# PeterFWS/Structure-PLP-SLAM

Measured on AMD Instinct MI355X. Metric: frames/sec ORB+LSD extract+match, 640x480 TUM-RGBD, 1/2/4/8 GPU, higher is better.
Workload: dtype u8

## Files before the change

### structure-plp-slam_amd/csrc/orb_context.hip

```cpp
#include <hip/hip_runtime.h>

#include <algorithm>
#include <cstdio>
#include <cstring>
#include <mutex>
#include <string>
#include <vector>

#include "blur_tile.hpp"
#include "orb_device.hpp"
#include "xcd_map.hpp"
#include "plp_common.hpp"
#include "quadtree_model.hpp"

namespace plp {
void launch_quadtree(hipStream_t st, const LevelDev* d_lv, int n_levels, int n_cells_total, const uint32_t* cell_cand,
                     const int32_t* cell_count, int32_t* sel, int32_t* sel_count, int total_sel_cap, uint32_t* qt_scratch,
                     size_t qt_scratch_frame_stride, int32_t* status, int B, int max_quota);
size_t quadtree_scratch_bytes_per_frame(const LevelDev* h_lv, int n_levels);
}

using namespace plp;

struct plp_orb {
    HostPinned pin;
    plp_orb_params p{};
    std::vector<float> rects;
    int device = 0;
    hipStream_t stream = nullptr;
    OrbScaleTables st;
    OrbGeometry geo;
    std::vector<LevelDev> h_lv;
    int total_blur_tiles = 0;
    DevBuf d_lv, d_cells, d_rs;
    ResizeDev rs{};
    int capB = 0;
    DevBuf pyr, blur, l0copy, cell_cand, cell_count, sel, sel_count, status, qt_scratch, d_mask;
    size_t l0copy_frame_stride = 0, qt_frame_stride = 0;
    int max_quota = 0;
    DevBuf s_kps, s_desc, s_counts;
    DevBuf stereo_corr, stereo_stage;
    int s_cap = 0;
    bool mask_is_initialized = false;
    std::vector<uint8_t> rect_mask;
    int rect_mask_rows = 0, rect_mask_cols = 0;
    bool rect_mask_uploaded = false;
    DevBuf d_rect_mask;
    int last_B = 0;
    OrbPlanes last_planes{};
    hipStream_t last_stream = nullptr;
    bool profiling = false;
    hipEvent_t ev[8] = {};
    double stage_ms[7] = {0, 0, 0, 0, 0, 0, 0};
    long stage_batches = 0;
    std::mutex mu;
};

namespace {

plp_status validate(const plp_orb_params* p) {
    if (!p) return set_error(PLP_ERR_INVALID_ARG, "params is NULL");
    if (p->num_levels == 0 || p->num_levels > (uint32_t)kMaxLevels) return set_error(PLP_ERR_INVALID_ARG, "num_levels must be in [1,16]");
    if (!(p->scale_factor > 1.0f)) return set_error(PLP_ERR_INVALID_ARG, "scale_factor must be > 1");
    if (p->n_mask_rects < 0 || (p->n_mask_rects > 0 && !p->mask_rects)) return set_error(PLP_ERR_INVALID_ARG, "mask_rects");
    for (int i = 0; i < p->n_mask_rects; ++i) {
        const float* v = p->mask_rects + 4 * i;
        if (v[0] >= v[1]) return set_error(PLP_ERR_INVALID_ARG, "x_max must be greater than x_min");
        if (v[2] >= v[3]) return set_error(PLP_ERR_INVALID_ARG, "y_max must be greater than x_min");
    }
    return PLP_OK;
}

void reinitialize(plp_orb* c) {
    c->st = make_scale_tables(c->p.max_num_keypts, c->p.scale_factor, c->p.num_levels);
    c->geo = OrbGeometry{};
}

plp_status build_geometry_impl(plp_orb* c, int rows, int cols);

plp_status build_geometry(plp_orb* c, int rows, int cols) {
    if (c->geo.rows == rows && c->geo.cols == cols && c->geo.n_levels == (int)c->p.num_levels) return PLP_OK;
    const plp_status s = build_geometry_impl(c, rows, cols);
    if (s != PLP_OK) { c->geo = OrbGeometry{}; c->h_lv.clear(); c->capB = 0; }
    return s;
}

plp_status build_geometry_impl(plp_orb* c, int rows, int cols) {
    const int nl = (int)c->p.num_levels;
    {
        OrbGeometry g = make_geometry(rows, cols, c->st, nl);
        for (int l = 0; l < nl; ++l)
            if (g.lv[l].w <= 2 * kOrbBorder + 6 || g.lv[l].h <= 2 * kOrbBorder + 6)
                return set_error(PLP_ERR_INVALID_ARG, "image too small for the requested pyramid (level narrower than 45 px)");
        if (cols - 2 * kOrbBorder > 4095 || rows - 2 * kOrbBorder > 4095)
            return set_error(PLP_ERR_UNSUPPORTED, "images larger than 4133 px are not supported (12-bit candidate packing)");
        c->geo = std::move(g);
    }
    c->h_lv.assign(nl, LevelDev{});
    c->total_blur_tiles = 0;
    size_t qt_off = 0;
    int max_cells = 0;
    for (int l = 0; l < nl; ++l) {
        const LevelGeom& G = c->geo.lv[l];
        LevelDev& L = c->h_lv[l];
        L.w = G.w; L.h = G.h; L.pitch = G.pitch; L.off = G.off;
        L.blur_tiles = ((G.w + 127) / 128) * ((G.h + plp::kBlurTH - 1) / plp::kBlurTH);
        L.blur_tiles_x_magic = plp::plp_div_magic((uint32_t)((G.w + 127) / 128), (uint64_t)L.blur_tiles);
        c->total_blur_tiles += L.blur_tiles;
        L.scale = c->st.sf[l];
        L.sel_base = G.sel_base; L.sel_cap = G.sel_cap;
        L.cell_base = G.cell_base; L.n_cells = G.n_cell_rows * G.n_cell_cols;
        L.quota = (int)c->st.quota[l];
        c->max_quota = l == 0 ? L.quota : std::max(c->max_quota, L.quota);
        L.n_init_x = G.n_init_x; L.delta_x = G.delta_x; L.delta_y = G.delta_y;
        L.qt_cap = std::min(std::max(L.n_cells, 1) * kCellCap, 65535);
        L.qt_off = qt_off;
        qt_off += (size_t)L.qt_cap * 20;
        const int extent = (int)std::ceil(std::max(G.delta_x, G.delta_y)) + 1;
        int t1 = 0;
        while ((1 << t1) < extent) ++t1;
        const int d_eff = std::min(t1 + 2, kQtDepth);
        const int n_init = G.n_init_x * G.n_init_y;
        int nb = 0;
        while ((1 << nb) < n_init) ++nb;
        L.sort_lo = 2 * (kQtDepth - d_eff);
        L.sort_hi = 2 * kQtDepth + nb;
        if (L.n_cells > 2048 || 3 * L.quota + 8 > kQtMaxNodesLdsSmallBlock || n_init > 32)
            return set_error(PLP_ERR_UNSUPPORTED, "frame/keypoint budget exceeds the quadtree kernel limits (quota per level <= 2010, 2048 cells per level, 32 initial nodes)");
        max_cells = std::max(max_cells, L.n_cells);
    }
    if (3 * c->max_quota + 8 > kQtMaxNodesLds && max_cells > 1024)
        return set_error(PLP_ERR_UNSUPPORTED, "frame/keypoint budget exceeds the quadtree kernel limits (a quota above 1960 per level needs levels of at most 1024 cells)");
    PLP_HIP(c->d_lv.upload(c->h_lv.data(), sizeof(LevelDev) * nl, c->stream));
    PLP_HIP(c->d_cells.upload(c->geo.cells.data(), sizeof(CellDesc) * c->geo.cells.size(), c->stream));
    const ResizeTables& R = c->geo.rs;
    const size_t nc = R.xofs0.size(), nr = R.yofs0.size();
    std::vector<int16_t> blob;
    blob.reserve(4 * nc + 4 * nr + 8);
    auto push = [&](const std::vector<int16_t>& v) { size_t o = blob.size(); blob.insert(blob.end(), v.begin(), v.end()); return o; };
    const size_t o0 = push(R.xofs0), o1 = push(R.xofs1), o2 = push(R.a0), o3 = push(R.a1);
    const size_t o4 = push(R.yofs0), o5 = push(R.yofs1), o6 = push(R.b0), o7 = push(R.b1);
    if (blob.empty()) blob.push_back(0);
    PLP_HIP(c->d_rs.upload(blob.data(), blob.size() * 2, c->stream));
    const int16_t* base = (const int16_t*)c->d_rs.p;
    c->rs.xofs0 = base + o0; c->rs.xofs1 = base + o1; c->rs.a0 = base + o2; c->rs.a1 = base + o3;
    c->rs.yofs0 = base + o4; c->rs.yofs1 = base + o5; c->rs.b0 = base + o6; c->rs.b1 = base + o7;
    for (int l = 0; l < nl; ++l) { c->rs.col_base[l] = R.col_base[l]; c->rs.row_base[l] = R.row_base[l]; }
    c->capB = 0;
    PLP_HIP(hipStreamSynchronize(c->stream));
    return PLP_OK;
}

plp_status ensure_capacity(plp_orb* c, int B) {
    if (B <= c->capB) return PLP_OK;
    const OrbGeometry& g = c->geo;
    const size_t n_cells = g.cells.size();
    c->l0copy_frame_stride = ((size_t)g.lv[0].pitch * g.rows + 255) / 256 * 256;
    c->qt_frame_stride = quadtree_scratch_bytes_per_frame(c->h_lv.data(), g.n_levels);
    PLP_HIP(c->pyr.reserve(g.frame_plane_bytes * B));
    PLP_HIP(c->blur.reserve(g.frame_plane_bytes * B));
    PLP_HIP(c->l0copy.reserve(c->l0copy_frame_stride * B));
    PLP_HIP(c->cell_cand.reserve(sizeof(uint32_t) * kCellCap * n_cells * B));
    PLP_HIP(c->cell_count.reserve(sizeof(int32_t) * n_cells * B));
    PLP_HIP(c->sel.reserve(sizeof(int32_t) * g.total_sel_cap * B));
    PLP_HIP(c->sel_count.reserve(sizeof(int32_t) * kMaxLevels * B));
    PLP_HIP(c->status.reserve(sizeof(int32_t) * 4));
    PLP_HIP(c->qt_scratch.reserve(c->qt_frame_stride * B));
    c->capB = B;
    return PLP_OK;
}

void build_rect_mask(plp_orb* c, int rows, int cols) {
    if (c->mask_is_initialized || c->rects.empty()) return;
    if (c->rect_mask.empty()) { c->rect_mask.assign((size_t)rows * cols, 255); c->rect_mask_rows = rows; c->rect_mask_cols = cols; }
    for (size_t i = 0; i + 3 < c->rects.size(); i += 4) {
        const unsigned x0 = (unsigned)std::round((float)cols * c->rects[i]), x1 = (unsigned)std::round((float)cols * c->rects[i + 1]);
        const unsigned y0 = (unsigned)std::round((float)rows * c->rects[i + 2]), y1 = (unsigned)std::round((float)rows * c->rects[i + 3]);
        for (unsigned y = y0; y <= y1 && y < (unsigned)c->rect_mask_rows; ++y)
            for (unsigned x = x0; x <= x1 && x < (unsigned)c->rect_mask_cols; ++x) c->rect_mask[(size_t)y * c->rect_mask_cols + x] = 0;
    }
    c->mask_is_initialized = true;
    c->rect_mask_uploaded = false;
}

plp_status run_batch(plp_orb* c, const uint8_t* d_imgs, int B, int rows, int cols, size_t step, size_t frame_stride,
                     const uint8_t* d_mask, size_t mask_step, size_t mask_frame_stride, plp_keypoint* d_kps, uint8_t* d_desc,
                     int cap, int32_t* d_counts, hipStream_t st) {
    PLP_HIP(hipSetDevice(c->device));
    PLP_TRY(build_geometry(c, rows, cols));
    PLP_TRY(ensure_capacity(c, B));
    const OrbGeometry& g = c->geo;
    const int nl = g.n_levels;

    const bool prof = c->profiling;
    auto mark = [&](int i) { if (prof) (void)hipEventRecord(c->ev[i], st); };
    mark(0);
    OrbPlanes pl{};
    pl.pyr = (uint8_t*)c->pyr.p; pl.pyr_frame_stride = g.frame_plane_bytes;
    const bool aligned = ((uintptr_t)d_imgs % 4 == 0) && (step % 4 == 0) && (frame_stride % 4 == 0);
    if (aligned) { pl.l0 = d_imgs; pl.l0_frame_stride = frame_stride; pl.l0_pitch = (int)step; }
    else {
        for (int f = 0; f < B; ++f)
            PLP_HIP(hipMemcpy2DAsync((uint8_t*)c->l0copy.p + f * c->l0copy_frame_stride, g.lv[0].pitch, d_imgs + f * frame_stride, step,
                                     cols, rows, hipMemcpyDeviceToDevice, st));
        pl.l0 = (const uint8_t*)c->l0copy.p; pl.l0_frame_stride = c->l0copy_frame_stride; pl.l0_pitch = g.lv[0].pitch;
    }
    build_rect_mask(c, rows, cols);
    if (!d_mask && !c->rect_mask.empty()) {
        if (c->rect_mask_rows != rows || c->rect_mask_cols != cols)
            return set_error(PLP_ERR_INVALID_ARG, "rectangle mask was built for a different frame size");
        if (!c->rect_mask_uploaded) {
            PLP_HIP(c->d_rect_mask.upload(c->rect_mask.data(), c->rect_mask.size(), st));
            c->rect_mask_uploaded = true;
        }
        d_mask = (const uint8_t*)c->d_rect_mask.p; mask_step = cols; mask_frame_stride = 0;
    }

    PLP_HIP(hipMemsetAsync(c->status.p, 0, 16, st));
    mark(1);
    for (int l = 1; l < nl; ++l) launch_resize(st, pl, c->h_lv.data(), l, B, c->rs);
    mark(2);
    launch_fast(st, pl, (const CellDesc*)c->d_cells.p, (int)g.cells.size(), (const LevelDev*)c->d_lv.p, B, (int)c->p.ini_fast_thr,
                (int)c->p.min_fast_thr, d_mask, mask_step, mask_frame_stride, (uint32_t*)c->cell_cand.p, (int32_t*)c->cell_count.p);
    mark(3);
    BlurTaps taps{{18, 34, 48, 56, 48, 34, 18}};
    launch_blur(st, pl, (uint8_t*)c->blur.p, g.frame_plane_bytes, (const LevelDev*)c->d_lv.p, nl, c->total_blur_tiles, B, taps, c->h_lv.data());
    mark(4);
    launch_quadtree(st, (const LevelDev*)c->d_lv.p, nl, (int)g.cells.size(), (const uint32_t*)c->cell_cand.p,
                    (const int32_t*)c->cell_count.p, (int32_t*)c->sel.p, (int32_t*)c->sel_count.p, g.total_sel_cap,
                    (uint32_t*)c->qt_scratch.p, c->qt_frame_stride, (int32_t*)c->status.p, B, c->max_quota);
    mark(5);
    UMax um;
    for (int v = 0; v <= kHalfPatch; ++v) um.v[v] = c->st.u_max[v];
    launch_orient_rbrief(st, pl, (const uint8_t*)c->blur.p, g.frame_plane_bytes, (const LevelDev*)c->d_lv.p, nl, (const int32_t*)c->sel.p,
                         (const int32_t*)c->sel_count.p, g.total_sel_cap, um, d_kps, d_desc, cap, d_counts, (int32_t*)c->status.p, B);
    PLP_HIP(hipGetLastError());
    if (prof) {
        mark(6);
        PLP_HIP(hipEventSynchronize(c->ev[6]));
        for (int i = 0; i < 6; ++i) { float ms = 0; PLP_HIP(hipEventElapsedTime(&ms, c->ev[i], c->ev[i + 1])); c->stage_ms[i] += ms; }
        float tot = 0; PLP_HIP(hipEventElapsedTime(&tot, c->ev[0], c->ev[6])); c->stage_ms[6] += tot;
        ++c->stage_batches;
    }
    c->last_B = B; c->last_planes = pl; c->last_stream = st;
    return PLP_OK;
}

}

extern "C" {

void plp_orb_default_params(plp_orb_params* p) {
    if (!p) return;
    p->max_num_keypts = 2000; p->scale_factor = 1.2f; p->num_levels = 8; p->ini_fast_thr = 20; p->min_fast_thr = 7;
    p->mask_rects = nullptr; p->n_mask_rects = 0;
}

plp_status plp_orb_create(const plp_orb_params* params, int device, plp_orb** out) {
    if (!out) return set_error(PLP_ERR_INVALID_ARG, "out is NULL");
    *out = nullptr;
// ... 292 lines not shown
```

### structure-plp-slam_amd/csrc/orb_device.hpp

```cpp
#pragma once
#include <hip/hip_runtime.h>
#include <stdint.h>

#include "../../include/plp_front.h"
#include "orb_tables.hpp"

namespace plp {

constexpr int kQtMaxNodesLds = 5888;
constexpr int kQtMaxNodesLdsSmallBlock = 6040;

struct LevelDev {
    int w, h, pitch;
    int blur_tiles;
    uint32_t blur_tiles_x_magic;
    size_t off;
    float scale;
    int sel_base, sel_cap;
    int cell_base, n_cells;
    int quota;
    int n_init_x;
    double delta_x, delta_y;
    size_t qt_off;
    int qt_cap;
    int sort_lo, sort_hi;
};

struct OrbPlanes {
    const uint8_t* l0; size_t l0_frame_stride; int l0_pitch;
    uint8_t* pyr; size_t pyr_frame_stride;
    __host__ __device__ const uint8_t* level_ptr(int frame, int level, const LevelDev& L) const {
        return level == 0 ? l0 + (size_t)frame * l0_frame_stride : pyr + (size_t)frame * pyr_frame_stride + L.off;
    }
    __host__ __device__ int level_pitch(int level, const LevelDev& L) const { return level == 0 ? l0_pitch : L.pitch; }
};

struct BlurTaps { int k[7]; };
struct UMax { int v[kHalfPatch + 1]; };

struct ResizeDev {
    const int16_t *xofs0, *xofs1, *a0, *a1, *yofs0, *yofs1, *b0, *b1;
    int col_base[kMaxLevels], row_base[kMaxLevels];
};

struct StereoArgs {
    const plp_keypoint *kps_l, *kps_r;
    const uint8_t *desc_l, *desc_r;
    const int32_t *cnt_l, *cnt_r;
    int cap;
    float fxb, tb;
    float inv_scale[kMaxLevels];
    float* x_right; float* depth;
    int32_t* corr;
};
void launch_stereo(hipStream_t st, const OrbPlanes& pl_l, const OrbPlanes& pl_r, const LevelDev* d_lv, const StereoArgs& A, int B);

void launch_resize(hipStream_t st, const OrbPlanes& pl, const LevelDev* h_lv, int level, int B, const ResizeDev& rs);
void launch_fast(hipStream_t st, const OrbPlanes& pl, const CellDesc* d_cells, int n_cells, const LevelDev* d_lv, int B,
                 int ini_thr, int min_thr, const uint8_t* d_mask, size_t mask_step, size_t mask_frame_stride,
                 uint32_t* cell_cand, int32_t* cell_count);
void launch_blur(hipStream_t st, const OrbPlanes& pl, uint8_t* blur, size_t blur_frame_stride, const LevelDev* d_lv,
                 int n_levels, int total_tiles, int B, const BlurTaps& taps, const LevelDev* h_lv = nullptr);
void launch_orient_rbrief(hipStream_t st, const OrbPlanes& pl, const uint8_t* blur, size_t blur_frame_stride,
                          const LevelDev* d_lv, int n_levels, const int32_t* sel, const int32_t* sel_count,
                          int total_sel_cap, const UMax& um, plp_keypoint* kps, uint8_t* desc, int cap, int32_t* counts,
                          int32_t* status, int B);

}
```

### structure-plp-slam_amd/csrc/orb_kernels.hip

```cpp
#include <hip/hip_runtime.h>
#include <stdint.h>

#include "blur_tile.hpp"
#include "plp_barrier.hpp"
#include "orb_device.hpp"
#include "plp_common.hpp"
#include "xcd_map.hpp"

namespace plp {

__device__ __forceinline__ int rs_tab(const int16_t* __restrict__ t, int i) { return *reinterpret_cast<const int16_t*>(reinterpret_cast<const char*>(t) + ((uint32_t)i << 1)); }
constexpr int kRsRows = 44, kRsPitch = 96;

__global__ __launch_bounds__(256) __attribute__((amdgpu_waves_per_eu(7, 8))) void k_resize_linear(const uint8_t* __restrict__ src_base, size_t src_frame_stride,
                                                       int src_pitch, int sw, uint8_t* __restrict__ dst_base,
                                                       size_t dst_frame_stride, int dst_pitch, int dw, int dh,
                                                       const int16_t* __restrict__ xofs0, const int16_t* __restrict__ xofs1,
                                                       const int16_t* __restrict__ a0, const int16_t* __restrict__ a1,
                                                       const int16_t* __restrict__ yofs0, const int16_t* __restrict__ yofs1,
                                                       const int16_t* __restrict__ b0, const int16_t* __restrict__ b1) {
    constexpr int ROWS = 8;
    __shared__ __attribute__((aligned(16))) uint8_t tiles[4 * kRsRows * kRsPitch];
    const int lane = threadIdx.x & 63, wv = __builtin_amdgcn_readfirstlane((int)(threadIdx.x >> 6));
    const int strip_x0 = blockIdx.x * 64, strip_y0 = (blockIdx.y * 4 + wv) * 32;
    if (strip_y0 >= dh) return;
    uint8_t* tile = tiles + wv * (kRsRows * kRsPitch);
    const int strip_x1 = min(strip_x0 + 64, dw) - 1, strip_y1 = min(strip_y0 + 32, dh) - 1;
    const uint8_t* src = src_base + (size_t)blockIdx.z * src_frame_stride;
    uint8_t* dst = dst_base + (size_t)blockIdx.z * dst_frame_stride;
    const int xs = (int)xofs0[strip_x0] & ~15, xe = xofs1[strip_x1];
    const int ys = yofs0[strip_y0], ye = yofs1[strip_y1];
    const int nrows = ye - ys + 1, nchunks = (xe - xs) / 16 + 1;
    const bool staged = nrows <= kRsRows && nchunks * 16 <= kRsPitch;
    if (staged) {
        const bool wide = (((uintptr_t)src | (uintptr_t)src_pitch) & 15) == 0;
        const int c = lane & 7, r0 = lane >> 3;
        if (c < nchunks) {
            const int x = xs + 16 * c;
            if (wide && x + 16 <= src_pitch) {
                constexpr int NT = (kRsRows + 7) / 8;
                uint4 v[NT];
#pragma unroll
                for (int q = 0; q < NT; ++q) v[q] = *reinterpret_cast<const uint4*>(src + (uint32_t)(__mul24(ys + min(r0 + 8 * q, nrows - 1), src_pitch) + x));
#pragma unroll
                for (int q = 0; q < NT; ++q) { const int r = r0 + 8 * q; if (r < nrows) *reinterpret_cast<uint4*>(tile + r * kRsPitch + 16 * c) = v[q]; }
            } else
                for (int r = r0; r < nrows; r += 8) {
                    const uint8_t* g = src + (size_t)(ys + r) * src_pitch + x;
                    uint8_t* t = tile + r * kRsPitch + 16 * c;
                    for (int k = 0; k < 16; ++k) t[k] = x + k < sw ? g[k] : (uint8_t)0;
                }
        }
        __builtin_amdgcn_fence(__ATOMIC_ACQ_REL, "workgroup");
        __builtin_amdgcn_wave_barrier();
    }
    const int dy0 = strip_y0 + (lane >> 4) * ROWS;
    const int dx0 = strip_x0 + (lane & 15) * 4;
    if (dy0 >= dh || dx0 >= dw) return;
    int x0[4], x1[4], wa0[4], wa1[4];
#pragma unroll
    for (int i = 0; i < 4; ++i) {
        const int dx = min(dx0 + i, dw - 1);
        x0[i] = rs_tab(xofs0, dx); x1[i] = rs_tab(xofs1, dx); wa0[i] = rs_tab(a0, dx); wa1[i] = rs_tab(a1, dx);
    }
    if (staged) {
#pragma unroll
        for (int i = 0; i < 4; ++i) { x0[i] -= xs; x1[i] -= xs; }
        int cached_row = -1, hc[4] = {0, 0, 0, 0};
        auto hrow = [&](int y, int (&h)[4]) {
            const uint8_t* S = tile + (y - ys) * kRsPitch;
#pragma unroll
            for (int i = 0; i < 4; ++i) h[i] = S[x0[i]] * wa0[i] + S[x1[i]] * wa1[i];
        };
        uint32_t tyy[ROWS], tbb[ROWS];
#pragma unroll
        for (int r = 0; r < ROWS; ++r) {
            const int dy = min(dy0 + r, dh - 1);
            tyy[r] = (uint32_t)(uint16_t)rs_tab(yofs0, dy) | ((uint32_t)(uint16_t)rs_tab(yofs1, dy) << 16);
            tbb[r] = (uint32_t)(uint16_t)rs_tab(b0, dy) | ((uint32_t)(uint16_t)rs_tab(b1, dy) << 16);
        }
#pragma unroll
        for (int r = 0; r < ROWS; ++r) {
            const int dy = dy0 + r;
            if (dy >= dh) break;
            const int y0 = (int)(tyy[r] & 0xffffu), y1 = (int)(tyy[r] >> 16);
            const int wb0 = (int)(int16_t)(tbb[r] & 0xffffu), wb1 = (int)(int16_t)(tbb[r] >> 16);
            int h0[4], h1[4];
            if (y0 == cached_row) {
#pragma unroll
                for (int i = 0; i < 4; ++i) h0[i] = hc[i];
            } else hrow(y0, h0);
            if (y1 == y0) {
#pragma unroll
                for (int i = 0; i < 4; ++i) h1[i] = h0[i];
            } else hrow(y1, h1);
            uint32_t packed = 0;
#pragma unroll
            for (int i = 0; i < 4; ++i) {
                const int v = (((wb0 * (h0[i] >> 4)) >> 16) + ((wb1 * (h1[i] >> 4)) >> 16) + 2) >> 2;
                packed |= (uint32_t)(v & 255) << (8 * i);
                hc[i] = h1[i];
            }
            cached_row = y1;
            *reinterpret_cast<uint32_t*>(dst + (uint32_t)(__mul24(dy, dst_pitch) + dx0)) = packed;
        }
        return;
    }
    for (int r = 0; r < ROWS; ++r) {
        const int dy = dy0 + r;
        if (dy >= dh) break;
        const uint8_t* S0 = src + (size_t)yofs0[dy] * src_pitch;
        const uint8_t* S1 = src + (size_t)yofs1[dy] * src_pitch;
        const int wb0 = b0[dy], wb1 = b1[dy];
        uint32_t packed = 0;
#pragma unroll
        for (int i = 0; i < 4; ++i) {
            const int h0 = S0[x0[i]] * wa0[i] + S0[x1[i]] * wa1[i];
            const int h1 = S1[x0[i]] * wa0[i] + S1[x1[i]] * wa1[i];
            const int v = (((wb0 * (h0 >> 4)) >> 16) + ((wb1 * (h1 >> 4)) >> 16) + 2) >> 2;
            packed |= (uint32_t)(v & 255) << (8 * i);
        }
        *reinterpret_cast<uint32_t*>(dst + (size_t)dy * dst_pitch + dx0) = packed;
    }
}

constexpr int kFastQ1 = 1536, kFastQ2 = 512;
constexpr int kTileW = 76;
constexpr int kScoreW = 68;

__device__ __forceinline__ int min3(int a, int b, int c) { return min(a, min(b, c)); }

__global__ __launch_bounds__(256) __attribute__((amdgpu_waves_per_eu(8, 8))) void k_fast_cells(OrbPlanes pl, const CellDesc* __restrict__ cells,
                                                    const LevelDev* __restrict__ lv, int ini_thr, int min_thr,
                                                    const uint8_t* __restrict__ mask, size_t mask_step,
                                                    size_t mask_frame_stride, uint32_t* __restrict__ cell_cand,
                                                    int32_t* __restrict__ cell_count, int n_cells, uint32_t gx_magic) {
    __shared__ __attribute__((aligned(16))) uint8_t tile[70 * kTileW];
    __shared__ __attribute__((aligned(16))) uint8_t score[66 * kScoreW];
    __shared__ unsigned long long keepbits[64];
    __shared__ uint16_t queue[kFastQ1], queue2[kFastQ2];
    __shared__ unsigned long long bits1[64], bits2[64];
    __shared__ int q_count, q2_count, n_ini, wave_tot[4], run_base;

    unsigned ucell, uframe;
    xcd_frame_major(ucell, uframe, gx_magic);
    const int tid = threadIdx.x, frame = (int)uframe, cell = (int)ucell;
    const CellDesc cd = cells[cell];
    const LevelDev L = lv[cd.level];
    const int out_slot = frame * n_cells + cell;
    const float sf = L.scale;

    const uint8_t* mk = mask ? mask + (size_t)frame * mask_frame_stride : nullptr;
    auto masked = [&](int y, int x) -> bool {
        return mk[(size_t)(int)((float)y * sf) * mask_step + (int)((float)x * sf)] == 0;
    };
    if (mk) {
// ... 40 lines not shown
            const uint32_t U = *(reinterpret_cast<const uint32_t*>(&tile[ty * kTileW]) + (tx4 >> 2) + 1);
            const uint32_t D = *(reinterpret_cast<const uint32_t*>(&tile[(ty + 6) * kTileW]) + (tx4 >> 2) + 1);
#pragma unroll
            for (int k = 0; k < 4; ++k) {
                if (tx4 + k >= tw) break;
                const int v = (int)((C >> (8 * k)) & 255u);
                const int hi = v + thr, lo = v - thr;
                const int p0 = (int)((D >> (8 * k)) & 255u), p4 = (int)((Rq >> (8 * k)) & 255u), p8 = (int)((U >> (8 * k)) & 255u),
                          p12 = (int)((Lq >> (8 * k)) & 255u);
                const bool b0 = p0 > hi, b4 = p4 > hi, b8 = p8 > hi, b12 = p12 > hi;
                const bool d0 = p0 < lo, d4 = p4 < lo, d8 = p8 < lo, d12 = p12 < lo;
                if (((b0 | b8) & (b4 | b12)) | ((d0 | d8) & (d4 | d12))) {
                    atomicOr(&bits1[ty], 1ull << (tx4 + k));
                    const int slot = atomicAdd(&q_count, 1);
                    if (slot < kFastQ1) queue[slot] = (uint16_t)((ty << 6) | (tx4 + k));
                }
            }
        }
        wg_barrier();
        const int nq1 = q_count;
        const bool dense1 = nq1 <= kFastQ1;
        for (int j = tid; j < (dense1 ? nq1 : 4096); j += 256) {
            const int i = dense1 ? (int)queue[j] : j;
            const int ty = i >> 6, tx = i & 63;
            if (!dense1 && !((bits1[ty] >> tx) & 1ull)) continue;
            const uint8_t* c = &tile[(ty + 3) * kTileW + tx + 4];
            const int v = c[0];
            const int hi = v + thr, lo = v - thr;
            uint32_t B = 0, D = 0;
#define PLP_T(k, dx, dy) { const int p = c[(dy) * kTileW + (dx)]; B |= (uint32_t)(p > hi) << k; D |= (uint32_t)(p < lo) << k; }
            PLP_T(0, 0, 3) PLP_T(1, 1, 3) PLP_T(2, 2, 2) PLP_T(3, 3, 1) PLP_T(4, 3, 0) PLP_T(5, 3, -1) PLP_T(6, 2, -2) PLP_T(7, 1, -3)
            PLP_T(8, 0, -3) PLP_T(9, -1, -3) PLP_T(10, -2, -2) PLP_T(11, -3, -1) PLP_T(12, -3, 0) PLP_T(13, -3, 1) PLP_T(14, -2, 2) PLP_T(15, -1, 3)
#undef PLP_T
            auto arc9 = [](uint32_t m) -> bool {
                m |= m << 16;
                uint32_t x = m & (m >> 1);
                x &= x >> 2;
                x &= x >> 4;
                x &= m >> 8;
                return (x & 0xffffu) != 0;
            };
            if (arc9(B) || arc9(D)) {
                atomicOr(&bits2[ty], 1ull << tx);
                const int slot = atomicAdd(&q2_count, 1);
                if (slot < kFastQ2) queue2[slot] = (uint16_t)i;
            }
        }
        wg_barrier();
        const int nq = q2_count;
        const bool dense2 = nq <= kFastQ2;
        for (int j = tid; j < (dense2 ? nq : 4096); j += 256) {
            const int i = dense2 ? (int)queue2[j] : j;
            const int ty = i >> 6, tx = i & 63;
            if (!dense2 && !((bits2[ty] >> tx) & 1ull)) continue;
            const uint8_t* c = &tile[(ty + 3) * kTileW + tx + 4];
            const int v = c[0];
            typedef short v2s __attribute__((ext_vector_type(2)));
            auto pair = [&](int o_lo, int o_hi) -> v2s { v2s r; r.x = (short)((int)c[o_lo] - v); r.y = (short)((int)c[o_hi] - v); return r; };
            auto sw = [](v2s x) -> v2s { return __builtin_shufflevector(x, x, 1, 0); };
            v2s P[8];
            P[0] = pair(3 * kTileW, -3 * kTileW);          P[1] = pair(3 * kTileW + 1, -3 * kTileW - 1);
            P[2] = pair(2 * kTileW + 2, -2 * kTileW - 2);  P[3] = pair(kTileW + 3, -kTileW - 3);
            P[4] = pair(3, -3);                            P[5] = pair(-kTileW + 3, kTileW - 3);
            P[6] = pair(-2 * kTileW + 2, 2 * kTileW - 2);  P[7] = pair(-3 * kTileW + 1, 3 * kTileW - 1);
            v2s n2[8], x2[8];
#pragma unroll
            for (int k = 0; k < 8; ++k) {
                const v2s nxt = k < 7 ? P[k + 1] : sw(P[0]);
                n2[k] = __builtin_elementwise_min(P[k], nxt); x2[k] = __builtin_elementwise_max(P[k], nxt);
            }
            v2s n4[8], x4[8];
#pragma unroll
            for (int k = 0; k < 8; ++k) {
                n4[k] = __builtin_elementwise_min(n2[k], k < 6 ? n2[k + 2] : sw(n2[k - 6]));
                x4[k] = __builtin_elementwise_max(x2[k], k < 6 ? x2[k + 2] : sw(x2[k - 6]));
            }
            v2s br, dk;
#pragma unroll
            for (int k = 0; k < 8; ++k) {
                const v2s d8 = sw(P[k]);
                const v2s mn9 = __builtin_elementwise_min(__builtin_elementwise_min(n4[k], k < 4 ? n4[k + 4] : sw(n4[k - 4])), d8);
                const v2s mx9 = __builtin_elementwise_max(__builtin_elementwise_max(x4[k], k < 4 ? x4[k + 4] : sw(x4[k - 4])), d8);
                br = k ? __builtin_elementwise_max(br, mn9) : mn9;
                dk = k ? __builtin_elementwise_min(dk, mx9) : mx9;
            }
            const int bright = max((int)br.x, (int)br.y), dark = min((int)dk.x, (int)dk.y);
            const int sc = max(bright, -dark) - 1;
            score[(ty + 1) * kScoreW + tx + 1] = (uint8_t)(sc >= thr ? sc : 0);
        }
        wg_barrier();
        int my_ini = 0;
        for (int j = tid; j < (dense2 ? nq : 4096); j += 256) {
            const int i = dense2 ? (int)queue2[j] : j;
            const int ty = i >> 6, tx = i & 63;
            if (!dense2 && !((bits2[ty] >> tx) & 1ull)) continue;
            const uint8_t* sp = &score[(ty + 1) * kScoreW + tx + 1];
            const int v = sp[0];
            const bool ok = v > 0 && v > sp[-1] && v > sp[1] && v > sp[-kScoreW - 1] && v > sp[-kScoreW] && v > sp[-kScoreW + 1] &&
                            v > sp[kScoreW - 1] && v > sp[kScoreW] && v > sp[kScoreW + 1];
            if (ok) { atomicOr(&keepbits[ty], 1ull << tx); ++my_ini; }
        }
        if (my_ini) atomicAdd(&n_ini, my_ini);
        wg_barrier();
        const int found = n_ini;
        wg_barrier();
        if (found > 0 || min_thr >= ini_thr) break;
    }

    uint32_t* out = cell_cand + (size_t)out_slot * kCellCap;
    const int lane = tid & 63, wv = tid >> 6;
    if (!mk) {
        if (wv != 0) return;
        unsigned long long m = keepbits[lane];
        const int cnt = __popcll(m);
        int inc = cnt;
#pragma unroll
        for (int o = 1; o < 64; o <<= 1) { const int t = __shfl_up(inc, o); if (lane >= o) inc += t; }
        int pos = inc - cnt;
        const uint32_t y = (uint32_t)(lane + 3 + cd.cy * kCellSize);
        while (m) {
            const int tx = __builtin_ctzll(m);
            m &= m - 1;
            const uint32_t v = score[(lane + 1) * kScoreW + tx + 1];
            if (pos < kCellCap) out[pos] = (uint32_t)(tx + 3 + cd.cx * kCellSize) | (y << 12) | (v << 24);
            ++pos;
        }
        if (lane == 63) cell_count[out_slot] = inc;
        return;
    }
    auto row_mask = [&](int ty) -> unsigned long long {
        const unsigned long long m = keepbits[ty];
        return __ballot(((m >> lane) & 1ull) && !masked(cd.min_y + ty + 3, cd.min_x + lane + 3));
    };
    int cnt = 0;
    for (int ty = 16 * wv; ty < 16 * wv + 16; ++ty) cnt += __popcll(row_mask(ty));
    if (lane == 0) wave_tot[wv] = cnt;
    wg_barrier();
    int off = 0;
    for (int k = 0; k < wv; ++k) off += wave_tot[k];
    for (int ty = 16 * wv; ty < 16 * wv + 16; ++ty) {
        const unsigned long long m = row_mask(ty);
        if ((m >> lane) & 1ull) {
            const uint32_t v = score[(ty + 1) * kScoreW + lane + 1];
            const uint32_t x = (uint32_t)(lane + 3 + cd.cx * kCellSize), y = (uint32_t)(ty + 3 + cd.cy * kCellSize);
            out[off + __popcll(m & ((1ull << lane) - 1ull))] = x | (y << 12) | (v << 24);
        }
        off += __popcll(m);
    }
    if (tid == 0) run_base = wave_tot[0] + wave_tot[1] + wave_tot[2] + wave_tot[3];
    wg_barrier();
    if (tid == 0) cell_count[out_slot] = run_base;
}

__global__ __launch_bounds__(256) __attribute__((amdgpu_waves_per_eu(8, 8))) void k_blur7(OrbPlanes pl, uint8_t* __restrict__ blur_base, size_t blur_frame_stride,
                                               const LevelDev* __restrict__ lv, int n_levels, BlurTaps taps, uint32_t gx_magic) {
    __shared__ BlurTileLds<3> S;
    unsigned ut, uf;
    xcd_frame_major(ut, uf, gx_magic);
    int t = (int)ut;
    const int frame = (int)uf;
    int level = 0;
    while (level + 1 < n_levels && t >= lv[level].blur_tiles) { t -= lv[level].blur_tiles; ++level; }
    const LevelDev L = lv[level];
    const int tiles_x = (L.w + kBlurTW - 1) / kBlurTW;
    const int trow = (int)plp_div((unsigned)t, (unsigned)tiles_x, L.blur_tiles_x_magic);
    blur_tile<3>(S, pl.level_ptr(frame, level, L), pl.level_pitch(level, L), blur_base + (size_t)frame * blur_frame_stride + L.off, L.pitch,
                 L.w, L.h, (t - trow * tiles_x) * kBlurTW, trow * kBlurTH, taps.k);
}

__device__ __forceinline__ float fast_atan2_deg(float y, float x) {
    const float p1 = 0.9997878412794807f * (float)(180 / 3.14159265358979323846);
    const float p3 = -0.3258083974640975f * (float)(180 / 3.14159265358979323846);
    const float p5 = 0.1555786518463281f * (float)(180 / 3.14159265358979323846);
    const float p7 = -0.04432655554792128f * (float)(180 / 3.14159265358979323846);
    const float eps = (float)2.2204460492503131e-16;
    const float ax = fabsf(x), ay = fabsf(y);
    float a;
    if (ax >= ay) {
        const float c = __fdiv_rn(ay, __fadd_rn(ax, eps));
        const float c2 = __fmul_rn(c, c);
        a = __fmul_rn(__fadd_rn(__fmul_rn(__fadd_rn(__fmul_rn(__fadd_rn(__fmul_rn(p7, c2), p5), c2), p3), c2), p1), c);
    } else {
        const float c = __fdiv_rn(ax, __fadd_rn(ay, eps));
        const float c2 = __fmul_rn(c, c);
        a = __fsub_rn(90.f, __fmul_rn(__fadd_rn(__fmul_rn(__fadd_rn(__fmul_rn(__fadd_rn(__fmul_rn(p7, c2), p5), c2), p3), c2), p1), c));
    }
    if (x < 0) a = __fsub_rn(180.f, a);
    if (y < 0) a = __fsub_rn(360.f, a);
    return a;
}

__device__ __forceinline__ float ref_poly_cos(float v) {
    const float v2 = __fmul_rn(v, v);
    return __fadd_rn(0.99940307f, __fmul_rn(v2, __fadd_rn(-0.49558072f, __fmul_rn(0.03679168f, v2))));
}
__device__ __forceinline__ float ref_cos(float v) {
    const float PI = 3.14159265358979f, PI_2 = PI / 2.0f, TWO_PI = 2.0f * PI, INV_TWO_PI = 1.0f / TWO_PI, THREE_PI_2 = 3.0f * PI_2;
    const float q = __fmul_rn(v, INV_TWO_PI);
    int fl = (int)q;
    fl -= (fl > q);
    v = __fsub_rn(v, __fmul_rn((float)fl, TWO_PI));
    v = (0.0f < v) ? v : -v;
    if (v < PI_2) return ref_poly_cos(v);
    if (v < PI) return -ref_poly_cos(__fsub_rn(PI, v));
    if (v < THREE_PI_2) return -ref_poly_cos(__fsub_rn(v, PI));
    return ref_poly_cos(__fsub_rn(TWO_PI, v));
}
__device__ __forceinline__ float ref_sin(float v) { return ref_cos(__fsub_rn(3.14159265358979f / 2.0f, v)); }

__constant__ __attribute__((aligned(16))) int8_t c_pattern[1024] = {
#include "rbrief_pattern.inc"
};

__device__ __forceinline__ uint32_t load_u32_unaligned(const uint8_t* p) {
    uint32_t v;
    __builtin_memcpy(&v, p, 4);
    return v;
}
__device__ __forceinline__ uint4 load_u128_unaligned(const uint8_t* p) {
    uint4 v;
    __builtin_memcpy(&v, p, 16);
    return v;
}
__device__ __forceinline__ int row16_sum(int v) {
    v += __builtin_amdgcn_update_dpp(v, v, 0x128, 0xf, 0xf, false);
    v += __builtin_amdgcn_update_dpp(v, v, 0x124, 0xf, 0xf, false);
    v += __builtin_amdgcn_update_dpp(v, v, 0x122, 0xf, 0xf, false);
    v += __builtin_amdgcn_update_dpp(v, v, 0x121, 0xf, 0xf, false);
    return v;
}

__global__ __launch_bounds__(256) void k_orient_rbrief(OrbPlanes pl, const uint8_t* __restrict__ blur_base,
                                                       size_t blur_frame_stride, const LevelDev* __restrict__ lv,
                                                       int n_levels, const int32_t* __restrict__ sel,
                                                       const int32_t* __restrict__ sel_count,
                                                       int total_sel_cap, UMax um, plp_keypoint* __restrict__ out_kps,
                                                       uint8_t* __restrict__ out_desc, int cap, int32_t* __restrict__ out_counts,
                                                       int32_t* __restrict__ status, uint32_t gx_magic) {
    __shared__ uint32_t s_w0[16][8], s_w1[16][8];
    __shared__ uint32_t s_pat[256];
    __shared__ __attribute__((aligned(16))) uint8_t s_patch[16 * 37 * 48];
    unsigned ublk, uframe;
    xcd_frame_major(ublk, uframe, gx_magic);
    const int tid = threadIdx.x, sub = tid & 15, frame = (int)uframe;
    const int32_t* cnt = sel_count + frame * kMaxLevels;
    int total = 0;
    for (int l = 0; l < n_levels; ++l) total += cnt[l];
    if (ublk == 0 && tid == 0) {
        out_counts[frame] = min(total, cap);
        if (total > cap) atomicOr(status, 1);
    }
    if ((int)ublk * 16 >= min(total, cap)) return;
    if (tid < 128) {
        const int av = tid >> 3, j = tid & 7, half = um.v[av];
        uint32_t w0 = 0, w1 = 0;
        for (int k = 0; k < 4; ++k) {
            const int u = 4 * j + k - 15;
            if (u <= 15 && (u < 0 ? -u : u) <= half) { w0 |= 1u << (8 * k); w1 |= (uint32_t)(u + 15) << (8 * k); }
        }
        s_w0[av][j] = w0; s_w1[av][j] = w1;
    }
    s_pat[tid] = reinterpret_cast<const uint32_t*>(c_pattern)[tid];
    wg_barrier();
    const int out_idx = (int)ublk * 16 + (tid >> 4);
    if (out_idx >= total || out_idx >= cap) return;
    int level = 0, i = out_idx;
    while (level + 1 < n_levels && i >= cnt[level]) { i -= cnt[level]; ++level; }
    const LevelDev L = lv[level];
    const int g = L.sel_base + i;

    const uint32_t pk = (uint32_t)sel[(size_t)frame * total_sel_cap + g];
    const int cx = (int)(pk & 0xfff) + kOrbBorder, cy = (int)((pk >> 12) & 0xfff) + kOrbBorder;
    const int resp = (int)(pk >> 24);
    if (cx < kOrbBorder || cy < kOrbBorder || cx > L.w - 1 - kOrbBorder || cy > L.h - 1 - kOrbBorder) {
        if (sub == 0) atomicOr(status, 8);
        return;
    }

    uint8_t* patch = s_patch + (tid >> 4) * (37 * 48);
    const uint8_t* img = pl.level_ptr(frame, level, L);
    const int pitch = pl.level_pitch(level, L);
    {
        const uint8_t* p0 = img + (size_t)(cy - 15) * pitch + cx - 15;
#pragma unroll
        for (int it = 0; it < 4; ++it) {
            const int item = sub + 16 * it, row = item >> 1, half = item & 1;
            if (row < 31) *reinterpret_cast<uint4*>(patch + row * 48 + 16 * half) = load_u128_unaligned(p0 + (size_t)row * pitch + 16 * half);
        }
    }
    __builtin_amdgcn_fence(__ATOMIC_ACQ_REL, "workgroup");
    __builtin_amdgcn_wave_barrier();
    int m10 = 0, m01 = 0;
    {
        const int vA = sub - 15, vB = sub + 1;
        const uint4* pA = reinterpret_cast<const uint4*>(patch + (vA + 15) * 48);
        const uint4* pB = reinterpret_cast<const uint4*>(patch + (min(vB, 15) + 15) * 48);
        const uint4 a0 = pA[0], a1 = pA[1], b0 = pB[0], b1 = pB[1];
        const uint32_t dA[8] = {a0.x, a0.y, a0.z, a0.w, a1.x, a1.y, a1.z, a1.w}, dB[8] = {b0.x, b0.y, b0.z, b0.w, b1.x, b1.y, b1.z, b1.w};
        uint32_t sA = 0, tA = 0, sB = 0, tB = 0;
        const int aA = -vA, aB = min(vB, 15);
#pragma unroll
        for (int j = 0; j < 8; ++j) {
            sA = __builtin_amdgcn_udot4(dA[j], s_w0[aA][j], sA, false); tA = __builtin_amdgcn_udot4(dA[j], s_w1[aA][j], tA, false);
            sB = __builtin_amdgcn_udot4(dB[j], s_w0[aB][j], sB, false); tB = __builtin_amdgcn_udot4(dB[j], s_w1[aB][j], tB, false);
        }
        if (vB > 15) { sB = 0; tB = 0; }
        m10 = (int)tA - 15 * (int)sA + (int)tB - 15 * (int)sB;
        m01 = vA * (int)sA + vB * (int)sB;
    }
    m10 = row16_sum(m10); m01 = row16_sum(m01);
    const float angle = fast_atan2_deg((float)m01, (float)m10);

    const float arad = (float)((double)angle * 3.14159265358979323846 / 180.0);
    const float ca = ref_cos(arad), sa = ref_sin(arad);
    __builtin_amdgcn_fence(__ATOMIC_ACQ_REL, "workgroup");
    __builtin_amdgcn_wave_barrier();
    {
        const uint8_t* b0 = blur_base + (size_t)frame * blur_frame_stride + L.off + (size_t)(cy - 18) * L.pitch + cx - 18;
#pragma unroll
        for (int it = 0; it < 7; ++it) {
            const int item = sub + 16 * it, row = item / 3, seg = item - 3 * row;
            if (row < 37) *reinterpret_cast<uint4*>(patch + row * 48 + 16 * seg) = load_u128_unaligned(b0 + (size_t)row * L.pitch + 16 * seg);
        }
    }
    __builtin_amdgcn_fence(__ATOMIC_ACQ_REL, "workgroup");
    __builtin_amdgcn_wave_barrier();
    const uint8_t* bl = patch + 18 * 48 + 18;
    uint32_t bits = 0;
    int ta[16], tb[16];
#pragma unroll
    for (int r = 0; r < 16; ++r) {
        const uint32_t pt = s_pat[16 * sub + r];
        const float ax = (float)(int8_t)(pt & 0xff), ay = (float)(int8_t)((pt >> 8) & 0xff), bx = (float)(int8_t)((pt >> 16) & 0xff),
                    by = (float)(int8_t)(pt >> 24);
        const int ar = __float2int_rn(__fadd_rn(__fmul_rn(ax, sa), __fmul_rn(ay, ca)));
        const int ac = __float2int_rn(__fsub_rn(__fmul_rn(ax, ca), __fmul_rn(ay, sa)));
        const int br = __float2int_rn(__fadd_rn(__fmul_rn(bx, sa), __fmul_rn(by, ca)));
        const int bc = __float2int_rn(__fsub_rn(__fmul_rn(bx, ca), __fmul_rn(by, sa)));
        ta[r] = bl[ar * 48 + ac]; tb[r] = bl[br * 48 + bc];
    }
#pragma unroll
    for (int r = 0; r < 16; ++r) bits |= (uint32_t)(ta[r] < tb[r]) << r;
    reinterpret_cast<uint16_t*>(out_desc + ((size_t)frame * cap + out_idx) * 32)[sub] = (uint16_t)bits;
    if (sub == 0) {
        plp_keypoint k;
        const float s = L.scale;
        k.x = level ? __fmul_rn((float)cx, s) : (float)cx;
        k.y = level ? __fmul_rn((float)cy, s) : (float)cy;
        k.size = (float)(unsigned)(__fmul_rn((float)kFastPatch, s));
        k.angle = angle;
        k.response = (float)resp;
        k.octave = level;
        k.class_id = -1;
        out_kps[(size_t)frame * cap + out_idx] = k;
    }
}

void launch_resize(hipStream_t st, const OrbPlanes& pl, const LevelDev* h_lv, int level, int B, const ResizeDev& rs) {
    const LevelDev& S = h_lv[level - 1];
    const LevelDev& D = h_lv[level];
    const uint8_t* src = level - 1 == 0 ? pl.l0 : pl.pyr + S.off;
    const size_t sstride = level - 1 == 0 ? pl.l0_frame_stride : pl.pyr_frame_stride;
    const int spitch = level - 1 == 0 ? pl.l0_pitch : S.pitch;
    dim3 grid((D.w + 63) / 64, (D.h + 127) / 128, B), block(256);
    hipLaunchKernelGGL(k_resize_linear, grid, block, 0, st, src, sstride, spitch, S.w, pl.pyr + D.off, pl.pyr_frame_stride, D.pitch,
                       D.w, D.h, rs.xofs0 + rs.col_base[level], rs.xofs1 + rs.col_base[level], rs.a0 + rs.col_base[level],
                       rs.a1 + rs.col_base[level], rs.yofs0 + rs.row_base[level], rs.yofs1 + rs.row_base[level],
                       rs.b0 + rs.row_base[level], rs.b1 + rs.row_base[level]);
}

void launch_fast(hipStream_t st, const OrbPlanes& pl, const CellDesc* d_cells, int n_cells, const LevelDev* d_lv, int B,
                 int ini_thr, int min_thr, const uint8_t* d_mask, size_t mask_step, size_t mask_frame_stride,
                 uint32_t* cell_cand, int32_t* cell_count) {
    hipLaunchKernelGGL(k_fast_cells, dim3(n_cells, B), dim3(256), 0, st, pl, d_cells, d_lv, ini_thr, min_thr, d_mask, mask_step,
                       mask_frame_stride, cell_cand, cell_count, n_cells, plp_div_magic((uint32_t)n_cells, (uint64_t)n_cells * B));
}

void launch_blur(hipStream_t st, const OrbPlanes& pl, uint8_t* blur, size_t blur_frame_stride, const LevelDev* d_lv,
                 int n_levels, int total_tiles, int B, const BlurTaps& taps, const LevelDev* h_lv) {
    (void)h_lv;
    hipLaunchKernelGGL(k_blur7, dim3(total_tiles, B), dim3(256), 0, st, pl, blur, blur_frame_stride, d_lv, n_levels, taps, plp_div_magic((uint32_t)total_tiles, (uint64_t)total_tiles * B));
}

void launch_orient_rbrief(hipStream_t st, const OrbPlanes& pl, const uint8_t* blur, size_t blur_frame_stride,
                          const LevelDev* d_lv, int n_levels, const int32_t* sel, const int32_t* sel_count,
                          int total_sel_cap, const UMax& um, plp_keypoint* kps, uint8_t* desc, int cap, int32_t* counts,
                          int32_t* status, int B) {
    hipLaunchKernelGGL(k_orient_rbrief, dim3((total_sel_cap + 15) / 16, B), dim3(256), 0, st, pl, blur, blur_frame_stride, d_lv,
                       n_levels, sel, sel_count, total_sel_cap, um, kps, desc, cap, counts, status,
                       plp_div_magic((uint32_t)((total_sel_cap + 15) / 16), (uint64_t)((total_sel_cap + 15) / 16) * B));
}

__global__ __launch_bounds__(256) void k_stereo_match(OrbPlanes pl_l, OrbPlanes pl_r, const LevelDev* __restrict__ lv, StereoArgs A) {
    const int lane = threadIdx.x & 63, b = blockIdx.y;
    const int il = blockIdx.x * 4 + __builtin_amdgcn_readfirstlane((int)(threadIdx.x >> 6));
    const int nl = A.cnt_l ? min(A.cnt_l[b], A.cap) : A.cap, nr = A.cnt_r ? min(A.cnt_r[b], A.cap) : A.cap;
    if (il >= A.cap) return;
    float* xr_out = A.x_right + (size_t)b * A.cap;
    float* dp_out = A.depth + (size_t)b * A.cap;
    int32_t* corr_out = A.corr + (size_t)b * A.cap;
    if (lane == 0) { xr_out[il] = -1.0f; dp_out[il] = -1.0f; corr_out[il] = -1; }
    if (il >= nl) return;
    const plp_keypoint kp = A.kps_l[(size_t)b * A.cap + il];
    const plp_keypoint* kr = A.kps_r + (size_t)b * A.cap;
    const float max_disp = __fdiv_rn(A.fxb, A.tb), min_disp = 0.0f;
    const int row = (int)(unsigned long long)kp.y;
    const float min_x = __fsub_rn(kp.x, max_disp), max_x = __fsub_rn(kp.x, min_disp);
    if (max_x < 0) return;
    const uint4* ql = reinterpret_cast<const uint4*>(A.desc_l + ((size_t)b * A.cap + il) * 32);
    const uint4 q0 = ql[0], q1 = ql[1];
    unsigned best = (75u << 16) | 0xffffu;
    for (int ir = lane; ir < nr; ir += 64) {
        const plp_keypoint k = kr[ir];
        const float r = __fmul_rn(2.0f, lv[k.octave].scale);
        const float lo = __fsub_rn(k.y, r), hi = __fadd_rn(k.y, r);
        int min_r = (int)lo; min_r -= (min_r > lo);
        int max_r = (int)hi; max_r += (max_r < hi);
        if (row < min_r || row > max_r) continue;
        if (k.octave < kp.octave - 1 || k.octave > kp.octave + 1) continue;
        if (k.x < min_x || max_x < k.x) continue;
        const uint4* d = reinterpret_cast<const uint4*>(A.desc_r + ((size_t)b * A.cap + ir) * 32);
        const uint4 d0 = d[0], d1 = d[1];
        const unsigned dist = __popc(q0.x ^ d0.x) + __popc(q0.y ^ d0.y) + __popc(q0.z ^ d0.z) + __popc(q0.w ^ d0.w) +
                              __popc(q1.x ^ d1.x) + __popc(q1.y ^ d1.y) + __popc(q1.z ^ d1.z) + __popc(q1.w ^ d1.w);
        best = min(best, (dist << 16) | (unsigned)ir);
    }
#pragma unroll
    for (int o = 32; o > 0; o >>= 1) best = min(best, (unsigned)__shfl_xor((int)best, o));
    if ((best >> 16) >= 75u) return;
    const plp_keypoint kpr = kr[best & 0xffffu];
    const LevelDev L = lv[kp.octave];
    const float isf = A.inv_scale[kp.octave];
    const int sxl = __float2int_rn(__fmul_rn(kp.x, isf)), syl = __float2int_rn(__fmul_rn(kp.y, isf)), sxr = __float2int_rn(__fmul_rn(kpr.x, isf));
    constexpr int win = 5, slide = 5;
    if (sxr - slide - win < 0 || L.w <= sxr + slide + win) return;
    const uint8_t* IL = pl_l.level_ptr(b, kp.octave, L);
    const uint8_t* IR = pl_r.level_ptr(b, kp.octave, L);
    const int pitch_l = pl_l.level_pitch(kp.octave, L), pitch_r = pl_r.level_pitch(kp.octave, L);
    const int lc = IL[(size_t)syl * pitch_l + sxl];
    int lv0 = 0, lv1 = 0;
    const int p0 = lane, p1 = lane + 64;
    const int dy0 = p0 / 11 - win, dx0 = p0 % 11 - win, dy1 = p1 / 11 - win, dx1 = p1 % 11 - win;
    lv0 = (int)IL[(size_t)(syl + dy0) * pitch_l + sxl + dx0] - lc;
    if (p1 < 121) lv1 = (int)IL[(size_t)(syl + dy1) * pitch_l + sxl + dx1] - lc;
    int corr[2 * slide + 1];
    int best_corr = 0x7fffffff, best_off = 0;
#pragma unroll
    for (int off = -slide; off <= slide; ++off) {
        const int rc = IR[(size_t)syl * pitch_r + sxr + off];
        int s = abs(lv0 - ((int)IR[(size_t)(syl + dy0) * pitch_r + sxr + off + dx0] - rc));
        if (p1 < 121) s += abs(lv1 - ((int)IR[(size_t)(syl + dy1) * pitch_r + sxr + off + dx1] - rc));
#pragma unroll
        for (int o = 32; o > 0; o >>= 1) s += __shfl_xor(s, o);
        corr[off + slide] = s;
        if (s < best_corr) { best_corr = s; best_off = off; }
    }
    if (best_off == -slide || best_off == slide) return;
    float c1 = 0, c2 = 0, c3 = 0;
#pragma unroll
    for (int i = 1; i < 2 * slide; ++i)
        if (i == best_off + slide) { c1 = (float)corr[i - 1]; c2 = (float)corr[i]; c3 = (float)corr[i + 1]; }
    const float x_delta = (float)((double)__fsub_rn(c1, c3) / (2.0 * (double)__fadd_rn(c1, c3) - 4.0 * (double)c2));
    if (x_delta < -1.0 || 1.0 < x_delta) return;
    float best_x_right = __fmul_rn(L.scale, __fadd_rn((float)(sxr + best_off), x_delta));
    float best_disp = __fsub_rn(kp.x, best_x_right);
    if (best_disp < min_disp || max_disp <= best_disp) return;
    if (best_disp <= 0.0f) { best_disp = 0.01f; best_x_right = __fsub_rn(kp.x, best_disp); }
    if (lane == 0) { dp_out[il] = __fdiv_rn(A.fxb, best_disp); xr_out[il] = best_x_right; corr_out[il] = best_corr; }
}

__global__ __launch_bounds__(256) void k_stereo_median(StereoArgs A) {
    __shared__ int hist[256], s_sel[3];
    const int tid = threadIdx.x, b = blockIdx.x;
    const int nl = A.cnt_l ? min(A.cnt_l[b], A.cap) : A.cap;
    int32_t* corr = A.corr + (size_t)b * A.cap;
    float* xr_out = A.x_right + (size_t)b * A.cap;
    float* dp_out = A.depth + (size_t)b * A.cap;
    hist[tid] = 0;
    wg_barrier();
    for (int i = tid; i < nl; i += 256) { const int c = corr[i]; if (c >= 0) atomicAdd(&hist[min(c >> 8, 255)], 1); }
    wg_barrier();
    if (tid == 0) {
        int total = 0;
        for (int i = 0; i < 256; ++i) total += hist[i];
        int k = total / 2, hb = 0;
        if (total) { while (k >= hist[hb]) { k -= hist[hb]; ++hb; } }
        s_sel[0] = total; s_sel[1] = hb; s_sel[2] = k;
    }
    wg_barrier();
    const int total = s_sel[0], hb = s_sel[1], k = s_sel[2];
    if (total == 0) return;
    wg_barrier();
    hist[tid] = 0;
    wg_barrier();
    for (int i = tid; i < nl; i += 256) { const int c = corr[i]; if (c >= 0 && min(c >> 8, 255) == hb) atomicAdd(&hist[c & 255], 1); }
    wg_barrier();
    if (tid == 0) {
        int kk = k, lb = 0;
        while (kk >= hist[lb]) { kk -= hist[lb]; ++lb; }
        s_sel[1] = (hb << 8) | lb;
    }
    wg_barrier();
    const float median = (float)s_sel[1];
    const float thr = (float)(2.0 * (double)median);
    for (int i = tid; i < nl; i += 256) { const int c = corr[i]; if (c >= 0 && thr < (float)c) { xr_out[i] = -1.0f; dp_out[i] = -1.0f; } }
}

void launch_stereo(hipStream_t st, const OrbPlanes& pl_l, const OrbPlanes& pl_r, const LevelDev* d_lv, const StereoArgs& A, int B) {
    hipLaunchKernelGGL(k_stereo_match, dim3((A.cap + 3) / 4, B), dim3(256), 0, st, pl_l, pl_r, d_lv, A);
    hipLaunchKernelGGL(k_stereo_median, dim3(B), dim3(256), 0, st, A);
}

}
```

Measured before the change: 91490.

## Rewrite 7x7 Gaussian blur as register-resident wave strips using dot4 and DPP

Replaces the LDS-tiled blur kernel with a per-wave vertical strip scheme: each wave handles a 248x64 strip, each lane owns 4 columns, horizontal taps use DPP lane shifts plus udot4, and vertical taps use udot2 over a rolling register window of row pairs. This drops LDS staging and barriers and packs the arithmetic into dot-product instructions. Edge strips take a templated path with byte-permute reflection handling. The cost is more complex edge logic, a risk of rounding mismatches, and higher register pressure.

```diff
diff --git a/structure-plp-slam_amd/csrc/orb_context.hip b/structure-plp-slam_amd/csrc/orb_context.hip
--- a/structure-plp-slam_amd/csrc/orb_context.hip
+++ b/structure-plp-slam_amd/csrc/orb_context.hip
@@ -7,7 +7,6 @@
 #include <string>
 #include <vector>
 
-#include "blur_tile.hpp"
 #include "orb_device.hpp"
 #include "xcd_map.hpp"
 #include "plp_common.hpp"
@@ -104,8 +103,8 @@
         const LevelGeom& G = c->geo.lv[l];
         LevelDev& L = c->h_lv[l];
         L.w = G.w; L.h = G.h; L.pitch = G.pitch; L.off = G.off;
-        L.blur_tiles = ((G.w + 127) / 128) * ((G.h + plp::kBlurTH - 1) / plp::kBlurTH);
-        L.blur_tiles_x_magic = plp::plp_div_magic((uint32_t)((G.w + 127) / 128), (uint64_t)L.blur_tiles);
+        L.blur_tiles = ((G.w + kBlur7W - 1) / kBlur7W) * ((G.h + kBlur7H - 1) / kBlur7H);
+        L.blur_tiles_x_magic = plp::plp_div_magic((uint32_t)((G.w + kBlur7W - 1) / kBlur7W), (uint64_t)L.blur_tiles);
         c->total_blur_tiles += L.blur_tiles;
         L.scale = c->st.sf[l];
         L.sel_base = G.sel_base; L.sel_cap = G.sel_cap;
diff --git a/structure-plp-slam_amd/csrc/orb_device.hpp b/structure-plp-slam_amd/csrc/orb_device.hpp
--- a/structure-plp-slam_amd/csrc/orb_device.hpp
+++ b/structure-plp-slam_amd/csrc/orb_device.hpp
@@ -9,6 +9,8 @@
 
 constexpr int kQtMaxNodesLds = 5888;
 constexpr int kQtMaxNodesLdsSmallBlock = 6040;
+
+constexpr int kBlur7W = 248, kBlur7H = 64;
 
 struct LevelDev {
     int w, h, pitch;
diff --git a/structure-plp-slam_amd/csrc/orb_kernels.hip b/structure-plp-slam_amd/csrc/orb_kernels.hip
--- a/structure-plp-slam_amd/csrc/orb_kernels.hip
+++ b/structure-plp-slam_amd/csrc/orb_kernels.hip
@@ -1,7 +1,6 @@
 #include <hip/hip_runtime.h>
 #include <stdint.h>
 
-#include "blur_tile.hpp"
 #include "plp_barrier.hpp"
 #include "orb_device.hpp"
 #include "plp_common.hpp"
@@ -348,20 +347,131 @@
     if (tid == 0) cell_count[out_slot] = run_base;
 }
 
+__device__ __forceinline__ uint32_t b7_dot2(uint32_t a, uint32_t b, uint32_t c) {
+    typedef unsigned short us2 __attribute__((ext_vector_type(2)));
+    return __builtin_amdgcn_udot2(__builtin_bit_cast(us2, a), __builtin_bit_cast(us2, b), c, false);
+}
+
+template <bool EDGE>
+__device__ __forceinline__ void blur7_strip(const uint8_t* __restrict__ src, int sp, uint8_t* __restrict__ dst, int dp, int w, int h, int x, int y0, int y1,
+                                            const int* __restrict__ k) {
+    const int lane = threadIdx.x & 63;
+    const uint32_t xl = (uint32_t)min(max(x, 0), (w - 1) & ~3);
+    const bool out_lane = lane >= 1 && lane <= 62 && x < w;
+    uint32_t tp[4][3];
+#pragma unroll
+    for (int e = 0; e < 4; ++e)
+#pragma unroll
+        for (int m = 0; m < 3; ++m) {
+            uint32_t v = 0;
+#pragma unroll
+            for (int b = 0; b < 4; ++b) {
+                const int i = 4 * m + b - e;
+                if (i >= 0 && i < 7) v |= (uint32_t)k[i] << (8 * b);
+            }
+            tp[e][m] = v;
+        }
+    uint32_t te[4], to[4];
+#pragma unroll
+    for (int j = 0; j < 4; ++j) {
+        te[j] = (uint32_t)k[2 * j] | (j < 3 ? (uint32_t)k[2 * j + 1] << 16 : 0u);
+        to[j] = (j > 0 ? (uint32_t)k[2 * j - 1] : 0u) | ((uint32_t)k[2 * j] << 16);
+    }
+    const int n = w - x;
+    const uint32_t selc = n == 1 ? 0x01020304u : n == 2 ? 0x03040504u : n == 3 ? 0x05060504u : 0x07060504u;
+    const uint32_t selr = n == 2 ? 0x0c0c0c02u : n == 3 ? 0x0c0c0304u : n == 4 ? 0x0c040506u : n == 5 ? 0x0c020304u : n == 6 ? 0x0c040504u : 0x07060504u;
+    const bool r_low = n >= 1 && n <= 4, left = x == 0;
+
+    auto load_row = [&](int y) -> uint32_t {
+        const int yy = y < 0 ? -y : y >= h ? 2 * (h - 1) - y : y;
+        return *reinterpret_cast<const uint32_t*>(src + (uint32_t)(yy * sp + xl));
+    };
+    auto hsum = [&](uint32_t c, uint32_t (&a)[4]) {
+        uint32_t l = (uint32_t)__builtin_amdgcn_update_dpp(0, (int)c, 0x138, 0xf, 0xf, false);
+        uint32_t r = (uint32_t)__builtin_amdgcn_update_dpp(0, (int)c, 0x130, 0xf, 0xf, false);
+        if (EDGE) {
+            const uint32_t r2 = __builtin_amdgcn_perm(r_low ? c : r, r_low ? l : c, selr);
+            const uint32_t c2 = __builtin_amdgcn_perm(c, l, selc);
+            l = left ? __builtin_amdgcn_perm(c, c, 0x0102030cu) : l;
+            c = c2; r = r2;
+        }
+        const uint32_t d[3] = {l, c, r};
+#pragma unroll
+        for (int o = 0; o < 4; ++o) {
+            const int s = 1 + o, q0 = s >> 2, e = s & 3;
+            uint32_t acc = 0;
+#pragma unroll
+            for (int m = 0; m < (e + 7 + 3) / 4; ++m) acc = __builtin_amdgcn_udot4(d[q0 + m], tp[e][m], acc, false);
+            a[o] = acc;
+        }
+    };
+    auto pair = [&](uint32_t ca, uint32_t cb, uint32_t (&p)[4]) {
+        uint32_t ha[4], hb[4];
+        hsum(ca, ha);
+        hsum(cb, hb);
+#pragma unroll
+        for (int o = 0; o < 4; ++o) p[o] = ha[o] | (hb[o] << 16);
+    };
+
+    uint32_t P[4][4], Q[4];
+    {
+        uint32_t c[6];
+#pragma unroll
+        for (int i = 0; i < 6; ++i) c[i] = load_row(y0 - 3 + i);
+#pragma unroll
+        for (int i = 0; i < 4; ++i) Q[i] = load_row(y0 + 3 + i);
+#pragma unroll
+        for (int j = 0; j < 3; ++j) pair(c[2 * j], c[2 * j + 1], P[j]);
+    }
+    for (int r0 = y0; r0 < y1; r0 += 8) {
+#pragma unroll
+        for (int s = 0; s < 4; ++s) {
+            const int r = r0 + 2 * s;
+            uint32_t* q = &Q[2 * (s & 1)];
+            const uint32_t ca = q[0], cb = q[1];
+            q[0] = load_row(r + 7); q[1] = load_row(r + 8);
+            pair(ca, cb, P[3]);
+            uint32_t ev[4], od[4];
+#pragma unroll
+            for (int o = 0; o < 4; ++o) {
+                uint32_t a = 32768u, b = 32768u;
+#pragma unroll
+                for (int j = 0; j < 4; ++j) { a = b7_dot2(P[j][o], te[j], a); b = b7_dot2(P[j][o], to[j], b); }
+                ev[o] = a; od[o] = b;
+            }
+            const uint32_t oe = __builtin_amdgcn_perm(ev[1], ev[0], 0x0c0c0602u) | __builtin_amdgcn_perm(ev[3], ev[2], 0x06020c0cu);
+            const uint32_t oo = __builtin_amdgcn_perm(od[1], od[0], 0x0c0c0602u) | __builtin_amdgcn_perm(od[3], od[2], 0x06020c0cu);
+            if (out_lane && r < y1) *reinterpret_cast<uint32_t*>(dst + (uint32_t)(__mul24(r, dp) + x)) = oe;
+            if (out_lane && r + 1 < y1) *reinterpret_cast<uint32_t*>(dst + (uint32_t)(__mul24(r + 1, dp) + x)) = oo;
+#pragma unroll
+            for (int j = 0; j < 3; ++j)
+#pragma unroll
+                for (int o = 0; o < 4; ++o) P[j][o] = P[j + 1][o];
+        }
+    }
+}
+
 __global__ __launch_bounds__(256) __attribute__((amdgpu_waves_per_eu(8, 8))) void k_blur7(OrbPlanes pl, uint8_t* __restrict__ blur_base, size_t blur_frame_stride,
-                                               const LevelDev* __restrict__ lv, int n_levels, BlurTaps taps, uint32_t gx_magic) {
-    __shared__ BlurTileLds<3> S;
-    unsigned ut, uf;
-    xcd_frame_major(ut, uf, gx_magic);
-    int t = (int)ut;
+                                               const LevelDev* __restrict__ lv, int n_levels, BlurTaps taps, uint32_t gx_magic, int n_strips) {
+    unsigned ub, uf;
+    xcd_frame_major(ub, uf, gx_magic);
+    int t = (int)ub * 4 + __builtin_amdgcn_readfirstlane((int)(threadIdx.x >> 6));
+    if (t >= n_strips) return;
     const int frame = (int)uf;
     int level = 0;
     while (level + 1 < n_levels && t >= lv[level].blur_tiles) { t -= lv[level].blur_tiles; ++level; }
     const LevelDev L = lv[level];
-    const int tiles_x = (L.w + kBlurTW - 1) / kBlurTW;
-    const int trow = (int)plp_div((unsigned)t, (unsigned)tiles_x, L.blur_tiles_x_magic);
-    blur_tile<3>(S, pl.level_ptr(frame, level, L), pl.level_pitch(level, L), blur_base + (size_t)frame * blur_frame_stride + L.off, L.pitch,
-                 L.w, L.h, (t - trow * tiles_x) * kBlurTW, trow * kBlurTH, taps.k);
+    const int w = L.w, h = L.h;
+    const int strips_x = (w + kBlur7W - 1) / kBlur7W;
+    const int srow = (int)plp_div((unsigned)t, (unsigned)strips_x, L.blur_tiles_x_magic);
+    const int x0 = (t - srow * strips_x) * kBlur7W, x = x0 + 4 * ((int)(threadIdx.x & 63) - 1);
+    const int y0 = srow * kBlur7H, y1 = min(y0 + kBlur7H, h);
+    const uint8_t* src = pl.level_ptr(frame, level, L);
+    uint8_t* dst = blur_base + (size_t)frame * blur_frame_stride + L.off;
+    if (x0 == 0 || x0 + kBlur7W + 8 > w)
+        blur7_strip<true>(src, pl.level_pitch(level, L), dst, L.pitch, w, h, x, y0, y1, taps.k);
+    else
+        blur7_strip<false>(src, pl.level_pitch(level, L), dst, L.pitch, w, h, x, y0, y1, taps.k);
 }
 
 __device__ __forceinline__ float fast_atan2_deg(float y, float x) {
@@ -575,7 +685,9 @@
 void launch_blur(hipStream_t st, const OrbPlanes& pl, uint8_t* blur, size_t blur_frame_stride, const LevelDev* d_lv,
                  int n_levels, int total_tiles, int B, const BlurTaps& taps, const LevelDev* h_lv) {
     (void)h_lv;
-    hipLaunchKernelGGL(k_blur7, dim3(total_tiles, B), dim3(256), 0, st, pl, blur, blur_frame_stride, d_lv, n_levels, taps, plp_div_magic((uint32_t)total_tiles, (uint64_t)total_tiles * B));
+    const int blocks = (total_tiles + 3) / 4;
+    hipLaunchKernelGGL(k_blur7, dim3(blocks, B), dim3(256), 0, st, pl, blur, blur_frame_stride, d_lv, n_levels, taps,
+                       plp_div_magic((uint32_t)blocks, (uint64_t)blocks * B), total_tiles);
 }
 
 void launch_orient_rbrief(hipStream_t st, const OrbPlanes& pl, const uint8_t* blur, size_t blur_frame_stride,
```

Measured after the change: 93300 (median of 6 runs). 1.02x the previous value.
